# chymaera96/GraFP

Measured on AMD Instinct MI355X. Metric: clips/sec contrastive step @ batch 1024, higher is better.
Workload: dtype bf16; 1 GPU; contrastive step at global batch 1024 (1024 pairs/GPU x 1 GPU, global negatives), 1 s clips @16 kHz, mel->kNN-graph->GNN->NT-Xent, fwd+bwd+Adam, random-init GraphEncoder-t (18.4M params); global_batch=1024, parallelism=dp1, k=3

## Files before the change

### grafp_amd/_lib.py

```python
import ctypes
import os
import subprocess

import torch

_HERE = os.path.dirname(os.path.abspath(__file__))
LIB_PATH = os.environ.get("GRAFP_HIP_LIB") or os.path.join(_HERE, "libgrafp_hip.so")
HEADER_PATH = os.path.join(os.path.dirname(_HERE), "include", "grafp_hip.h")

_c = ctypes
_P = _c.c_void_p
_I = _c.c_int
_L = _c.c_int64
_Z = _c.c_size_t
_F = _c.c_float

SIGNATURES = {
    "grafp_abi_version": (_I, []),
    "grafp_last_error": (_c.c_char_p, []),
    "grafp_logmel_f32": (_I, [_P, _L, _I, _I, _I, _I, _I, _P, _P, _P, _P, _P, _P, _P]),
    "grafp_unfold_segments_f32": (_I, [_P, _I, _I, _I, _I, _P, _P]),
    "grafp_stream_logmel_f32": (_I, [_P, _P, _P, _P, _P, _P, _P, _I, _I, _I, _I, _I, _I, _P, _P, _P, _P, _P, _P, _P]),
    "grafp_stream_segments_f32": (_I, [_P, _P, _P, _I, _I, _I, _I, _I, _I, _P, _P]),
    "grafp_peak_extract_fwd_f32": (_I, [_P, _I, _I, _I, _P, _P, _I, _I, _I, _I, _P, _P, _P, _P]),
    "grafp_peak_extract_bwd_f32": (_I, [_P, _I, _I, _I, _I, _I, _I, _I, _P, _P, _P, _P, _P, _P, _P, _Z, _P]),
    "grafp_peak_extract_bwd_workspace": (_Z, [_I, _I, _I, _I]),
    "grafp_knn_graph_workspace": (_Z, [_I, _I, _I]),
    "grafp_knn_normalize_f32": (_I, [_P, _I, _I, _I, _I, _P, _P, _P]),
    "grafp_knn_topk_f32": (_I, [_P, _P, _I, _I, _I, _I, _P, _P]),
    "grafp_knn_topk_i32": (_I, [_P, _P, _I, _I, _I, _I, _P, _P]),
    "grafp_knn_normalize_strided": (_I, [_P, _I, _L, _L, _I, _I, _I, _I, _P, _P, _P]),
    "grafp_knn_graph_f32": (_I, [_P, _I, _I, _I, _I, _I, _P, _P, _Z, _P]),
    "grafp_knn_pre_supported": (_I, [_I, _I, _I]),
    "grafp_knn_pre_workspace": (_Z, [_I, _I, _I]),
    "grafp_knn_graph_pre": (_I, [_P, _I, _L, _L, _I, _I, _I, _I, _I, _P, _I, _P, _Z, _P]),
    "grafp_knn_split_supported": (_I, [_I, _I, _I]),
    "grafp_knn_split_preferred": (_I, [_I, _I, _I]),
    "grafp_knn_split_workspace": (_Z, [_I, _I, _I]),
    "grafp_knn_split_preferred_for": (_I, [_I, _I, _I, _I]),
    "grafp_knn_split_workspace_for": (_Z, [_I, _I, _I, _I]),
    "grafp_knn_graph_split": (_I, [_P, _I, _L, _L, _I, _I, _I, _I, _P, _I, _P, _Z, _P, _P]),
    "grafp_mrconv_fwd_f32": (_I, [_P, _P, _I, _I, _I, _I, _P, _P]),
    "grafp_mrconv_bwd_f32": (_I, [_P, _P, _P, _I, _I, _I, _I, _P, _P]),
    "grafp_mrconv_fwd_strided": (_I, [_P, _I, _L, _L, _P, _I, _I, _I, _I, _P, _L, _L, _P]),
    "grafp_mrconv_bwd_strided": (_I, [_P, _I, _L, _L, _P, _P, _L, _L, _I, _I, _I, _I, _P, _P]),
    "grafp_mrconv_fwd_strided_i32": (_I, [_P, _I, _L, _L, _P, _I, _I, _I, _I, _P, _L, _L, _P]),
    "grafp_mrconv_bwd_strided_i32": (_I, [_P, _I, _L, _L, _P, _P, _L, _L, _I, _I, _I, _I, _P, _P]),
    "grafp_mrconv_arg_supported": (_I, [_I, _L, _L, _L, _L, _I, _I]),
    "grafp_mrconv_fwd_arg": (_I, [_P, _I, _L, _L, _P, _I, _I, _I, _I, _I, _P, _L, _L, _P, _P]),
    "grafp_mrconv_bwd_arg": (_I, [_P, _I, _P, _I, _P, _L, _L, _I, _I, _I, _I, _P, _L, _L, _P]),
    "grafp_mrconv_plan": (_I, [_I, _L, _L, _L, _L, _I, _I, _I, _I, _I, _I, _I, _P]),
    "grafp_stride2_taps_fwd": (_I, [_P, _I, _L, _I, _P, _P]),
    "grafp_stride2_taps_bwd": (_I, [_P, _I, _L, _I, _P, _P]),
    "grafp_bn_workspace": (_Z, [_I, _L]),
    "grafp_bn_fwd": (_I, [_P, _I, _I, _L, _I, _P, _P, _P, _P, _I, _F, _F, _F, _I, _P, _P, _P, _P, _P, _P, _Z, _P]),
    "grafp_bn_bwd": (_I, [_P, _P, _I, _I, _L, _I, _P, _P, _P, _P, _P, _I, _F, _I, _P, _P, _P, _P, _P, _Z, _P]),
    "grafp_bn_sync_bytes": (_Z, [_I, _L]),
    "grafp_bn_fwd_1pass": (_I, [_P, _I, _I, _L, _I, _P, _P, _P, _P, _I, _F, _F, _F, _I, _P, _P, _P, _P, _P, _P, _Z, _P, _I, _P]),
    "grafp_bn_bwd_1pass": (_I, [_P, _P, _I, _I, _L, _I, _P, _P, _P, _P, _P, _I, _F, _I, _P, _P, _P, _P, _P, _Z, _P, _I, _P]),
    "grafp_bn_plan": (_I, [_I, _I, _L, _I, _I, _I, _I, _I, _P]),
    "grafp_ivfpq_scan_f32": (_I, [_P, _I, _I, _P, _I, _P, _I, _P, _P, _P, _I, _P, _L, _P, _P, _P]),
    "grafp_pq_assign_f32": (_I, [_P, _L, _I, _I, _P, _P, _P, _I, _P, _P, _P]),
    "grafp_kmeans_workspace": (_Z, [_L, _I, _I, _I]),
    "grafp_kmeans_f32": (_I, [_P, _L, _I, _I, _P, _P, _P, _I, _I, _P, _P, _Z, _P]),
    "grafp_ivfpq_probe_f32": (_I, [_P, _I, _I, _P, _I, _I, _P, _P]),
    "grafp_ivfpq_search_f32": (_I, [_P, _I, _I, _P, _I, _P, _I, _P, _P, _P, _P, _I, _I, _P, _P, _P]),
    "grafp_debug_occupy": (_I, [_I, _I, _L, _P]),
    "grafp_conv1x1_gemm_supported": (_I, [_I, _I, _I, _L, _I]),
    "grafp_conv1x1_gemm_partials": (_I, [_I, _I, _I, _L, _I]),
    "grafp_conv1x1_gemm_plan": (_I, [_I, _I, _I, _L, _I, _P]),
    "grafp_conv1x1_gemm_bf16": (_I, [_P, _P, _I, _I, _I, _L, _I, _P, _I, _F, _P, _P, _P]),
    "grafp_conv1x1_gemm_affine_bf16": (_I, [_P, _P, _I, _I, _I, _L, _I, _P, _I, _F, _P, _P]),
    "grafp_conv1x1_gemm_cat_bf16": (_I, [_P, _P, _I, _P, _I, _I, _L, _P, _P]),
    "grafp_split_bf16_planes": (_I, [_P, _L, _P, _P, _P]),
    "grafp_conv1x1_gemm_split_f32": (_I, [_P, _P, _I, _I, _L, _P, _P]),
    "grafp_weights_prepare": (_I, [_P, _P, _I, _P]),
    "grafp_bn_finalize": (_I, [_P, _I, _I, _I, _L, _I, _P, _P, _P, _F, _F, _I, _P, _P, _P, _P, _P, _P]),
    "grafp_bn_affine_bf16": (_I, [_P, _I, _L, _I, _P, _P, _I, _F, _P, _P]),
    "grafp_bn_finalize_affine_bf16": (_I, [_P, _P, _I, _I, _I, _L, _I, _P, _P, _P, _F, _F, _P, _P, _P, _P, _P, _P, _I, _F, _P, _P]),
    "grafp_conv1x1_wgrad_workspace": (_Z, [_I, _I, _I, _L]),
    "grafp_conv1x1_wgrad_bf16": (_I, [_P, _P, _I, _I, _I, _L, _P, _P, _Z, _P]),
    "grafp_conv1x1_wgrad_pro_workspace": (_Z, [_I, _I, _I, _L, _I]),
    "grafp_conv1x1_wgrad_plan": (_I, [_I, _I, _I, _L, _I, _P]),
    "grafp_conv1x1_wgrad_pro_bf16": (_I, [_P, _P, _I, _I, _I, _L, _I, _P, _I, _F, _P, _P, _Z, _P]),
# ... 93 lines not shown
```

### grafp_amd/csrc/mrconv.hip

```cpp
#include <math.h>

#define GRAFP_STORE_FAMILY 3
#include "elemio.h"

namespace grafp {

constexpr int MR_THREADS = 256;

__device__ __forceinline__ int clampi(int64_t v, int n) {
    return v < 0 ? 0 : (v >= n ? n - 1 : (int)v);
}

template <typename T> constexpr int MR_NPAR = sizeof(T) == 4 ? 2 : 4;

__device__ __forceinline__ unsigned long long mr_fix_encode(float g, float scale) {
    const float v = __builtin_rintf(g * scale);
    const float hf = __builtin_truncf(v * 9.5367431640625e-7f);
    const float lf = __builtin_fmaf(hf, -1048576.0f, v);
    const int hi = (int)hf, lo = (int)lf;
    return ((unsigned long long)(unsigned)(hi + (lo >> 31)) << 32) | (unsigned long long)(unsigned)lo;
}
__device__ __forceinline__ float mr_fix_decode(unsigned long long a) {
    const int lo = (int)(unsigned)a;
    const int hi = (int)(unsigned)(a >> 32) - (lo >> 31);
    return (float)__builtin_fma((double)hi, 1048576.0, (double)lo);
}
struct MrScale {
    float scale, inv_scale;
    bool poisoned;
    __device__ __forceinline__ unsigned long long encode(float g) const { return mr_fix_encode(g, scale); }
    __device__ __forceinline__ float out(float base, unsigned long long acc) const {
        return poisoned ? NAN : base + mr_fix_decode(acc) * inv_scale;
    }
};
__device__ __forceinline__ void mr_scale_publish(unsigned m, unsigned *s_max, int tid) {
#pragma unroll
    for (int o = 32; o > 0; o >>= 1) m = max(m, (unsigned)__shfl_xor((int)m, o));
    if ((tid & 63) == 0) s_max[tid >> 6] = m;
}
__device__ __forceinline__ MrScale mr_scale_read(const unsigned *s_max) {
    const unsigned mbits = max(max(s_max[0], s_max[1]), max(s_max[2], s_max[3]));
    MrScale s;
    s.poisoned = mbits >= 0x7f800000u;
    int ex = 0;
    (void)frexpf(__uint_as_float(mbits), &ex);
    int sh = mbits ? 39 - ex : 0;
    sh = sh > 100 ? 100 : sh;
    s.scale = ldexpf(1.0f, sh);
    s.inv_scale = ldexpf(1.0f, -sh);
    return s;
}

__device__ __forceinline__ bool mr_first_max(int k, float v, float &best) {
    const bool wins = k == 0 || v > best;
    if (wins) best = v;
    return wins;
}

#define MR_WALK(V, tid, N, c, n)                    \
    int c = ((tid) * (V)) / (N), n = ((tid) * (V)) - c * (N)
#define MR_NEXT(V, N, c, n)                         \
    do {                                            \
        n += MR_THREADS * (V);                      \
        while (n >= (N)) { n -= (N); ++c; }         \
    } while (0)
// ... 289 lines not shown
#pragma unroll
        for (int it = 0; it < MRB_ITEMS; ++it) {
            if (pc[it] < cc) {
                const float *row = rows + pc[it] * N;
                float best[4] = {-INFINITY, -INFINITY, -INFINITY, -INFINITY};
                int bj[4];
                for (int k = 0; k < K; ++k) {
                    const int4 j4 = *reinterpret_cast<const int4 *>(sidx + k * N + pn[it]);
                    const int jj[4] = {j4.x, j4.y, j4.z, j4.w};
#pragma unroll
                    for (int e = 0; e < 4; ++e)
                        if (mr_first_max(k, row[jj[e]] - xi[it][e], best[e])) bj[e] = jj[e];
                }
                if (!fx.poisoned) {
#pragma unroll
                    for (int e = 0; e < 4; ++e)
                        atomicAdd(reinterpret_cast<unsigned long long *>(&acc[pc[it] * N + bj[e]]), fx.encode(godd[it][e]));
                }
            }
        }
        __syncthreads();
#pragma unroll
        for (int it = 0; it < MRB_ITEMS; ++it)
            if (pc[it] < cc) {
                float v[4];
#pragma unroll
                for (int e = 0; e < 4; ++e)
                    v[e] = fx.out(base[it][e], (unsigned long long)acc[pc[it] * N + pn[it] + e]);
                ElemIO<T>::store(db + (size_t)(c0 + pc[it]) * x_sc + pn[it], v, false);
            }
    }
}

template <typename T, typename I>
__global__ __launch_bounds__(MR_THREADS) void mrconv_bwd_a_kernel(const unsigned char *__restrict__ arg,
                                                                  const I *__restrict__ idx,
                                                                  const T *__restrict__ gout, int64_t g_sb,
                                                                  int64_t g_sc, T *__restrict__ dx, int64_t d_sb,
                                                                  int64_t d_sc, int C, int N, int K, int CC, int plain) {
    extern __shared__ __attribute__((aligned(16))) char smem[];
    __shared__ unsigned s_max[MR_THREADS / 64];
    const int b = blockIdx.y, tid = threadIdx.x;
    unsigned long long *acc = reinterpret_cast<unsigned long long *>(smem);
    int *sidx = reinterpret_cast<int *>(acc + MRB_SLAB);
    const int nslab = (C + CC - 1) / CC;
    int off[MRB_ITEMS], pn[MRB_ITEMS], pc[MRB_ITEMS];
    mr_pieces(tid, N, pc, pn);
#pragma unroll
    for (int it = 0; it < MRB_ITEMS; ++it) off[it] = pc[it] * N + pn[it];
    const T *ge_p[MRB_ITEMS];
    T *dx_p[MRB_ITEMS];
    const unsigned char *ar_p[MRB_ITEMS];
    const int64_t cstep = (int64_t)gridDim.x * CC;
#pragma unroll
    for (int it = 0; it < MRB_ITEMS; ++it) {
        const int64_t c = (int64_t)blockIdx.x * CC + pc[it];
        ge_p[it] = gout + (size_t)b * g_sb + (size_t)(2 * c) * g_sc + pn[it];
        dx_p[it] = dx + (size_t)b * d_sb + (size_t)c * d_sc + pn[it];
        ar_p[it] = arg + ((size_t)b * C + c) * (N / 4) + pn[it] / 4;
    }
    const int64_t ge_step = 2 * cstep * g_sc, dx_step = cstep * d_sc, ar_step = cstep * (N / 4);
    typedef typename ElemIO<T>::Raw4 Raw;
    constexpr int NPAR = MR_NPAR<T>;
    Raw pe[NPAR][MRB_ITEMS], po[NPAR][MRB_ITEMS];
    unsigned pa[NPAR][MRB_ITEMS];
    auto fetch = [&](int par, int slab) {
        const int cc = min(CC, C - slab * CC);
#pragma unroll
        for (int it = 0; it < MRB_ITEMS; ++it) {
            if (pc[it] < cc) {
                pe[par][it] = GRAFP_LD_ONCE(16, reinterpret_cast<const Raw *>(ge_p[it]));
                po[par][it] = GRAFP_LD_ONCE(16, reinterpret_cast<const Raw *>(ge_p[it] + g_sc));
                pa[par][it] = *ar_p[it];
            }
            ge_p[it] += ge_step;
            ar_p[it] += ar_step;
        }
    };
    int slab = blockIdx.x;
    const int G = gridDim.x;
#pragma unroll
    for (int par = 0; par < NPAR; ++par)
        if (slab + par * G < nslab) fetch(par, slab + par * G);
    stage_idx<I>(sidx, idx + (size_t)b * N * K, N, K, tid);
    while (slab < nslab) {
#pragma unroll
        for (int par = 0; par < NPAR; ++par) {
            if (slab < nslab) {
                const int cc = min(CC, C - slab * CC);
                __syncthreads();
                float godd[MRB_ITEMS][4], base[MRB_ITEMS][4];
                unsigned ak[MRB_ITEMS];
                unsigned m = 0;
#pragma unroll
                for (int it = 0; it < MRB_ITEMS; ++it)
                    if (pc[it] < cc) {
                        ak[it] = pa[par][it];
                        *reinterpret_cast<uint4 *>(acc + off[it]) = make_uint4(0, 0, 0, 0);
                        *reinterpret_cast<uint4 *>(acc + off[it] + 2) = make_uint4(0, 0, 0, 0);
                        float ge[4];
                        ElemIO<T>::unpack(pe[par][it], ge);
                        ElemIO<T>::unpack(po[par][it], godd[it]);
#pragma unroll
                        for (int e = 0; e < 4; ++e) {
                            base[it][e] = ge[e] - godd[it][e];
                            m = max(m, __float_as_uint(godd[it][e]) & 0x7fffffffu);
                        }
                    }
                mr_scale_publish(m, s_max, tid);
                __syncthreads();
                if (slab + NPAR * G < nslab) fetch(par, slab + NPAR * G);
                const MrScale fx = mr_scale_read(s_max);
                if (!fx.poisoned) {
#pragma unroll
                    for (int it = 0; it < MRB_ITEMS; ++it)
                        if (pc[it] < cc) {
                            unsigned long long *arow = acc + (off[it] - pn[it]);
                            int bj[4] = {0, 0, 0, 0};
                            for (int k = 0; k < K; ++k) {
                                const int4 j4 = *reinterpret_cast<const int4 *>(sidx + k * N + pn[it]);
                                const int jj[4] = {j4.x, j4.y, j4.z, j4.w};
#pragma unroll
                                for (int e = 0; e < 4; ++e) bj[e] = ((ak[it] >> (2 * e)) & 3u) == (unsigned)k ? jj[e] : bj[e];
                            }
#pragma unroll
                            for (int e = 0; e < 4; ++e) atomicAdd(arow + bj[e], fx.encode(godd[it][e]));
                        }
                }
                __syncthreads();
#pragma unroll
                for (int it = 0; it < MRB_ITEMS; ++it) {
                    if (pc[it] < cc) {
                        float v[4];
                        const uint4 a01 = *reinterpret_cast<const uint4 *>(acc + off[it]);
                        const uint4 a23 = *reinterpret_cast<const uint4 *>(acc + off[it] + 2);
                        const unsigned long long a[4] = {((unsigned long long)a01.y << 32) | a01.x,
                                                         ((unsigned long long)a01.w << 32) | a01.z,
                                                         ((unsigned long long)a23.y << 32) | a23.x,
                                                         ((unsigned long long)a23.w << 32) | a23.z};
#pragma unroll
                        for (int e = 0; e < 4; ++e) v[e] = fx.out(base[it][e], a[e]);
                        ElemIO<T>::store(dx_p[it], v, plain != 0);
                    }
                    dx_p[it] += dx_step;
                }
                slab += G;
            }
        }
    }
}

enum { MR_PATH_PERSISTENT = 0, MR_PATH_VEC4 = 1, MR_PATH_SCALAR = 2, MR_PATH_RECORD = 3 };
struct MrLaunch {
    int path;
    int items;
    int cc;
    int nslab, per_clip;
    size_t lds;
};
constexpr size_t MR_LDS_LIMIT = 160 * 1024;
constexpr int MR_FWD_ELEMS = 4096;
static_assert(MRB_SLAB <= MRP_SLAB, "a row that fits the backward slab fits the forward one");

static inline int mr_clamp_cc(int cc, int C) { return cc < 1 ? 1 : (cc > C ? C : cc); }

static int mr_choose(int64_t x_sb, int64_t x_sc, int64_t o_sb, int64_t o_sc, int N, int K, int C, int B,
                     bool aligned, bool backward, bool with_arg, MrLaunch *L) {
    const bool v4 = aligned && N % 4 == 0 && x_sb % 4 == 0 && x_sc % 4 == 0 && o_sb % 4 == 0 && o_sc % 4 == 0;
    const size_t edges = (size_t)K * N;
    const size_t lds_fwd_p = (MRP_SLAB + edges) * 4, lds_bwd_p = (3 * (size_t)MRB_SLAB + edges) * 4,
                 lds_bwd_a = (2 * (size_t)MRB_SLAB + edges) * 4;
    auto lds_generic = [&](int cc) {
        const size_t slab = (size_t)cc * N;
        return (backward ? 4 * ((slab + 1) & ~(size_t)1) + edges : slab + edges) * 4;
    };
    const bool record = with_arg && v4 && K <= 4 && N <= MRB_SLAB && lds_fwd_p <= MR_LDS_LIMIT && lds_bwd_a <= MR_LDS_LIMIT;
    const int slab = backward ? MRB_SLAB : MRP_SLAB;
    const size_t lds_p = !backward ? lds_fwd_p : (record ? lds_bwd_a : lds_bwd_p);
// ... 6 lines not shown
    }
    int items = 0, cc = mr_clamp_cc(MR_FWD_ELEMS / N, C);
    if (backward) {
        const int per_item = MR_THREADS * (v4 ? 4 : 1);
        items = N <= 2 * per_item ? 2 : 8;
        cc = mr_clamp_cc(items * per_item / N, C);
        GRAFP_REQUIRE((size_t)cc * N <= (size_t)items * per_item, "mrconv_bwd: N=%d exceeds the %d nodes a workgroup covers", N,
                      items * per_item);
        while (cc > 1 && lds_generic(cc) > MR_LDS_LIMIT) --cc;
    }
    GRAFP_REQUIRE(lds_generic(cc) <= MR_LDS_LIMIT, "mrconv_%s: N=%d K=%d needs %zu B of LDS (> 160 KiB)",
                  backward ? "bwd" : "fwd", N, K, lds_generic(cc));
    *L = {v4 ? MR_PATH_VEC4 : MR_PATH_SCALAR, items, cc, (C + cc - 1) / cc, (C + cc - 1) / cc, lds_generic(cc)};
    return GRAFP_OK;
}

static int mr_check_args(const char *op, bool pointers, int dtype, int B, int C, int N, int K) {
    GRAFP_REQUIRE(pointers, "%s: null pointer", op);
    GRAFP_REQUIRE(B > 0 && C > 0 && N > 0 && K > 0, "%s: bad shape B=%d C=%d N=%d K=%d", op, B, C, N, K);
    GRAFP_REQUIRE(dtype == GRAFP_F32 || dtype == GRAFP_BF16, "%s: dtype %d not in {f32, bf16}", op, dtype);
    return GRAFP_OK;
}

static bool mr_aligned(int dtype, const void *a, const void *b, const void *c = nullptr) {
    return (((uintptr_t)a | (uintptr_t)b | (uintptr_t)c) % (dtype == GRAFP_F32 ? 16 : 8)) == 0;
}

template <typename Kern, typename... Args>
static int mr_launch(const char *name, Kern kern, const MrLaunch &L, int B, grafp_stream_t stream, Args... args) {
    (void)hipFuncSetAttribute((const void *)kern, hipFuncAttributeMaxDynamicSharedMemorySize, (int)L.lds);
    hipLaunchKernelGGL(kern, dim3(L.per_clip, B), dim3(MR_THREADS), L.lds, (hipStream_t)stream, args...);
    GRAFP_CHECK_LAUNCH(name);
    return GRAFP_OK;
}

}

static int mrconv_fwd_impl(const char *op, const void *x, int dtype, int64_t x_sb, int64_t x_sc, const void *idx, int idx32,
                           int B, int C, int N, int K, void *out, int64_t o_sb, int64_t o_sc, grafp_stream_t stream,
                           unsigned char *arg = nullptr) {
    using namespace grafp;
    if (int e = mr_check_args(op, x && idx && out, dtype, B, C, N, K)) return e;
    MrLaunch L;
    if (int e = mr_choose(x_sb, x_sc, o_sb, o_sc, N, K, C, B, mr_aligned(dtype, x, out), false, arg != nullptr, &L)) return e;
    GRAFP_REQUIRE(!arg || L.path == MR_PATH_RECORD,
                  "mrconv_fwd_arg: shape / alignment outside grafp_mrconv_arg_supported (N=%d K=%d)", N, K);
    int rc = GRAFP_OK;
    for_elem_idx(dtype, idx32, [&](auto te, auto ti) {
        using T = typename decltype(te)::type;
        using I = typename decltype(ti)::type;
        if (L.path == MR_PATH_PERSISTENT || L.path == MR_PATH_RECORD) {
            const int plain = plain_stores((size_t)2 * B * C * N * sizeof(T), "GRAFP_MR_PLAIN_MAX_MB", 140);
            for_bool(arg != nullptr, [&](auto wk) {
                rc = mr_launch("mrconv_fwd_p_kernel", mrconv_fwd_p_kernel<T, I, decltype(wk)::value>, L, B, stream, (const T *)x,
                               x_sb, x_sc, (const I *)idx, (T *)out, o_sb, o_sc, C, N, K, L.cc, arg, plain);
            });
        } else {
            for_bool(L.path == MR_PATH_VEC4, [&](auto vec) {
                rc = mr_launch("mrconv_fwd_kernel", mrconv_fwd_kernel<T, decltype(vec)::value ? 4 : 1, I>, L, B, stream,
                               (const T *)x, x_sb, x_sc, (const I *)idx, (T *)out, o_sb, o_sc, C, N, K, L.cc);
            });
        }
    });
    return rc;
}

static int mrconv_bwd_impl(const char *op, const void *x, const unsigned char *arg, int dtype, int64_t x_sb, int64_t x_sc,
                           const void *idx, int idx32, const void *grad_out, int64_t g_sb, int64_t g_sc, int B, int C, int N,
                           int K, void *dx, grafp_stream_t stream) {
    using namespace grafp;
    if (int e = mr_check_args(op, (x || arg) && idx && grad_out && dx, dtype, B, C, N, K)) return e;
    MrLaunch L;
    if (int e = mr_choose(x_sb, x_sc, g_sb, g_sc, N, K, C, B, mr_aligned(dtype, x, grad_out, dx), true, arg != nullptr, &L)) return e;
    GRAFP_REQUIRE(!arg || L.path == MR_PATH_RECORD,
                  "mrconv_bwd_arg: shape / alignment outside grafp_mrconv_arg_supported (N=%d K=%d)", N, K);
    int rc = GRAFP_OK;
    for_elem_idx(dtype, idx32, [&](auto te, auto ti) {
        using T = typename decltype(te)::type;
        using I = typename decltype(ti)::type;
        if (L.path == MR_PATH_RECORD) {
            const int plain = plain_stores((size_t)B * C * N * sizeof(T), "GRAFP_MR_PLAIN_MAX_MB", 140);
            rc = mr_launch("mrconv_bwd_a_kernel", mrconv_bwd_a_kernel<T, I>, L, B, stream, arg, (const I *)idx,
                           (const T *)grad_out, g_sb, g_sc, (T *)dx, x_sb, x_sc, C, N, K, L.cc, plain);
        } else if (L.path == MR_PATH_PERSISTENT) {
            rc = mr_launch("mrconv_bwd_p_kernel", mrconv_bwd_p_kernel<T, I>, L, B, stream, (const T *)x, x_sb, x_sc,
                           (const I *)idx, (const T *)grad_out, g_sb, g_sc, (T *)dx, C, N, K, L.cc);
        } else {
            for_bool(L.path == MR_PATH_VEC4, [&](auto vec) {
                for_bool(L.items == 2, [&](auto two) {
                    rc = mr_launch("mrconv_bwd_kernel",
                                   mrconv_bwd_kernel<T, decltype(vec)::value ? 4 : 1, I, decltype(two)::value ? 2 : 8>, L, B,
                                   stream, (const T *)x, x_sb, x_sc, (const I *)idx, (const T *)grad_out, g_sb, g_sc, (T *)dx,
                                   C, N, K, L.cc);
                });
            });
        }
    });
    return rc;
}

extern "C" int grafp_mrconv_fwd_strided(const void *x, int dtype, int64_t x_sb, int64_t x_sc, const int64_t *idx, int B,
                                        int C, int N, int K, void *out, int64_t o_sb, int64_t o_sc,
                                        grafp_stream_t stream) {
    return mrconv_fwd_impl("mrconv_fwd", x, dtype, x_sb, x_sc, idx, 0, B, C, N, K, out, o_sb, o_sc, stream);
}
extern "C" int grafp_mrconv_fwd_strided_i32(const void *x, int dtype, int64_t x_sb, int64_t x_sc, const int32_t *idx,
                                            int B, int C, int N, int K, void *out, int64_t o_sb, int64_t o_sc,
                                            grafp_stream_t stream) {
    return mrconv_fwd_impl("mrconv_fwd", x, dtype, x_sb, x_sc, idx, 1, B, C, N, K, out, o_sb, o_sc, stream);
}
extern "C" int grafp_mrconv_bwd_strided(const void *x, int dtype, int64_t x_sb, int64_t x_sc, const int64_t *idx,
                                        const void *grad_out, int64_t g_sb, int64_t g_sc, int B, int C, int N, int K,
                                        void *dx, grafp_stream_t stream) {
    return mrconv_bwd_impl("mrconv_bwd", x, nullptr, dtype, x_sb, x_sc, idx, 0, grad_out, g_sb, g_sc, B, C, N, K, dx, stream);
}
extern "C" int grafp_mrconv_bwd_strided_i32(const void *x, int dtype, int64_t x_sb, int64_t x_sc, const int32_t *idx,
// ... 47 lines not shown
```

### grafp_amd/encoder/graph_encoder.py

```python
import contextlib

import torch
import torch.nn.functional as F
from torch import nn

from .. import ops
from ._dense import (bn_act, conv1x1, conv_bn_act, deferred_counters, deferred_norm, from_cbn, shortcut_token,
                     stride2_operands, to_cbn)
from .gcn_lib.torch_nn import act_layer
from .gcn_lib.torch_vertex import Grapher

_SIZES = {
    "t": ([2, 2, 6, 2], [64, 128, 256, 512]),
    "s": ([2, 2, 6, 2], [80, 160, 400, 640]),
    "m": ([2, 2, 16, 2], [96, 192, 384, 768]),
}


class Downsample(nn.Module):

    def __init__(self, in_dim=3, out_dim=768):
        super().__init__()
        self.conv = nn.Sequential(nn.Conv2d(in_dim, out_dim, 3, stride=2, padding=1), nn.BatchNorm2d(out_dim))

# ... 86 lines not shown
    @contextlib.contextmanager
    def one_weight_preparation(self):
        if self._lowp_hold is not None:
            yield
            return
        self._lowp_hold = False
        try:
            yield
        finally:
            self._lowp_hold = None

    def forward(self, x, views=1):
        x = to_cbn(x)
        g = int(views)
        if torch.is_autocast_enabled() and x.is_cuda:
            if self._lowp is None:
                self._lowp = ops.lowp_weights([m for m in self.modules() if isinstance(m, nn.Conv2d)
                                               and m.kernel_size == (1, 1) and m is not self.proj])
            if not self._lowp_hold:
                self._lowp.refresh(torch.get_autocast_dtype("cuda"))
                if self._lowp_hold is not None:
                    self._lowp_hold = True
        elif self._lowp is not None:
            self._lowp.clear()
        with deferred_counters():
            x = conv_bn_act(self.stem[0], self.stem[1], x, act=ops.ACT_LEAKY, slope=self.stem[2].negative_slope,
                            groups=g)
            for mod in self.backbone:
                if isinstance(mod, Downsample):
                    x = mod.forward_cbn(x, g)
                else:
                    x = mod[1].forward_cbn(mod[0].forward_cbn(x, g), g)
        with torch.autocast(x.device.type, enabled=False):
            pooled = x.float().mean(dim=2)
            w = self.proj.weight.reshape(self.proj.out_channels, -1)
            h = torch.mm(w.float(), pooled) + self.proj.bias.float().reshape(-1, 1)
        return h.t().contiguous()
```

### grafp_amd/ops.py

```python
import collections
import contextlib
import ctypes
import math
import os

import numpy as np
import torch
from torch.amp import custom_bwd, custom_fwd

from ._lib import check, lib

_vp = ctypes.c_void_p


def _require_gpu(*tensors):
    for t in tensors:
        if t is not None and not t.is_cuda:
            raise RuntimeError(
                "grafp_amd ops run only on a HIP device (MI355X): got a CPU tensor and there is no CPU "
                "fallback by design (the CPU restatement lives in oracle/ and is test infrastructure).")


def _p(t):
    return _vp(t.data_ptr()) if t is not None else None
# ... 664 lines not shown
                                               N, K, _p(out), o_sb, o_sc, _p(arg), _stream()), "mrconv_fwd_arg")
            ctx.save_for_backward(arg, idx)
            return out
        fwd = lib.grafp_mrconv_fwd_strided_i32 if idx.dtype == torch.int32 else lib.grafp_mrconv_fwd_strided
        with _timed("mrconv_fwd", (B, C, N, K)):
            check(fwd(_p(x), _DT[x.dtype], sb, sc, _p(idx), B, C, N, K, _p(out), o_sb, o_sc, _stream()), "mrconv_fwd")
        ctx.save_for_backward(x, idx)
        return out

    @staticmethod
    def backward(ctx, grad_out):
        x, idx = ctx.saved_tensors
        layout = ctx.layout
        B, C, N, shape, dtype = ctx.dims
        K = idx.shape[-1]
        g = grad_out.detach().to(dtype).contiguous()
        g_sb, g_sc = (2 * C * N, N) if layout == "bcn" else (N, B * N)
        sb, sc = (C * N, N) if layout == "bcn" else (N, B * N)
        if ctx.from_arg:
            dx = torch.empty(shape, dtype=dtype, device=g.device)
            with _timed("mrconv_bwd", (B, C, N, K)):
                check(lib.grafp_mrconv_bwd_arg(_p(x), _DT[dtype], _p(idx), int(idx.dtype == torch.int32), _p(g), g_sb,
                                               g_sc, B, C, N, K, _p(dx), sb, sc, _stream()), "mrconv_bwd_arg")
            return dx, None, None
        dx = torch.empty_like(x)
        with _timed("mrconv_bwd", (B, C, N, K)):
            bwd = lib.grafp_mrconv_bwd_strided_i32 if idx.dtype == torch.int32 else lib.grafp_mrconv_bwd_strided
            check(bwd(_p(x), _DT[x.dtype], sb, sc, _p(idx), _p(g), g_sb, g_sc, B, C, N, K, _p(dx), _stream()), "mrconv_bwd")
        return dx, None, None


def max_relative(x, idx, layout="bcn"):
    return _MaxRelative.apply(x, idx, layout)


ACT_NONE, ACT_RELU, ACT_LEAKY = 0, 1, 2


_BN_SYNC = {}


def _bn_sync(device, C, M):
    if switches.bn_two_pass:
        return None
    key = (device, _raw_stream(device.index if device.index is not None else _cur_device()))
    buf = _BN_SYNC.get(key)
    need = int(lib.grafp_bn_sync_bytes(C, M))
    if buf is None or buf.numel() * 8 < need:
        buf = torch.full((max(1 << 18, (need + 7) // 8),), -1, dtype=torch.int64, device=device)
        _BN_SYNC[key] = buf
    return buf


class _BnAct(torch.autograd.Function):
    @staticmethod
    def forward(ctx, x, gamma, beta, pre_bias, residual, running_mean, running_var, training, momentum, eps, act,
                slope, groups):
        _require_gpu(x, gamma, beta)
        if x.dtype not in _DT:
            x = x.float()
        x = x.detach().contiguous()
        C = x.shape[0]
        M = x.numel() // C
        res = None if residual is None else residual.detach().to(x.dtype).contiguous()
        g32, b32 = _f32c(gamma), _f32c(beta)
        pb = None if pre_bias is None else _f32c(pre_bias)
# ... 1482 lines not shown
```

### include/grafp_hip.h

```cpp
#ifndef GRAFP_HIP_H
#define GRAFP_HIP_H

#include <stddef.h>
#include <stdint.h>

#ifdef __cplusplus
extern "C" {
#endif

#define GRAFP_OK 0
#define GRAFP_ERR_ARG (-1)
#define GRAFP_ERR_WORKSPACE (-2)
#define GRAFP_ERR_LAUNCH (-3)

#define GRAFP_ABI_VERSION 1
#define GRAFP_KNN_MAX_K 8
#define GRAFP_SEARCH_MAX_K 32

typedef void *grafp_stream_t;

#define GRAFP_F32 0
#define GRAFP_BF16 1

int grafp_abi_version(void);
// ... 44 lines not shown

int grafp_knn_split_supported(int C, int N, int k);
int grafp_knn_split_preferred(int C, int N, int k);
int grafp_knn_split_preferred_for(int dtype, int C, int N, int k);
size_t grafp_knn_split_workspace(int B, int C, int N);
size_t grafp_knn_split_workspace_for(int dtype, int B, int C, int N);
int grafp_knn_graph_split(const void *x, int dtype, int64_t stride_b, int64_t stride_c, int B, int C, int N, int k,
                          void *idx, int idx_is_i32, void *ws, size_t ws_bytes, int32_t *n_uncertified,
                          grafp_stream_t stream);

int grafp_mrconv_fwd_f32(const float *x, const int64_t *idx, int B, int C, int N, int K, float *out,
                         grafp_stream_t stream);
int grafp_mrconv_bwd_f32(const float *x, const int64_t *idx, const float *grad_out, int B, int C, int N, int K,
                         float *dx, grafp_stream_t stream);
int grafp_mrconv_fwd_strided(const void *x, int dtype, int64_t x_sb, int64_t x_sc, const int64_t *idx, int B, int C,
                             int N, int K, void *out, int64_t o_sb, int64_t o_sc, grafp_stream_t stream);
int grafp_mrconv_bwd_strided(const void *x, int dtype, int64_t x_sb, int64_t x_sc, const int64_t *idx,
                             const void *grad_out, int64_t g_sb, int64_t g_sc, int B, int C, int N, int K, void *dx,
                             grafp_stream_t stream);

int grafp_mrconv_fwd_strided_i32(const void *x, int dtype, int64_t x_sb, int64_t x_sc, const int32_t *idx, int B, int C,
                                 int N, int K, void *out, int64_t o_sb, int64_t o_sc, grafp_stream_t stream);
int grafp_mrconv_bwd_strided_i32(const void *x, int dtype, int64_t x_sb, int64_t x_sc, const int32_t *idx,
                                 const void *grad_out, int64_t g_sb, int64_t g_sc, int B, int C, int N, int K,
                                 void *dx, grafp_stream_t stream);
int grafp_mrconv_arg_supported(int dtype, int64_t x_sb, int64_t x_sc, int64_t o_sb, int64_t o_sc, int N, int K);
int grafp_mrconv_fwd_arg(const void *x, int dtype, int64_t x_sb, int64_t x_sc, const void *idx, int idx_is_i32, int B,
                         int C, int N, int K, void *out, int64_t o_sb, int64_t o_sc, uint8_t *arg, grafp_stream_t stream);
int grafp_mrconv_bwd_arg(const uint8_t *arg, int dtype, const void *idx, int idx_is_i32, const void *grad_out,
                         int64_t g_sb, int64_t g_sc, int B, int C, int N, int K, void *dx, int64_t d_sb, int64_t d_sc,
                         grafp_stream_t stream);
int grafp_mrconv_plan(int dtype, int64_t x_sb, int64_t x_sc, int64_t o_sb, int64_t o_sc, int B, int C, int N, int K,
                      int aligned, int backward, int with_arg, int *info);

size_t grafp_bn_workspace(int C, int64_t M);
int grafp_bn_fwd(const void *x, int dtype, int C, int64_t M, int groups, const float *pre_bias, const float *gamma,
                 const float *beta, const void *residual, int act, float slope, float eps, float momentum,
                 int training, float *running_mean, float *running_var, void *out, float *save_mean,
                 float *save_invstd, void *ws, size_t ws_bytes, grafp_stream_t stream);
int grafp_bn_bwd(const void *x, const void *dz, int dtype, int C, int64_t M, int groups, const float *pre_bias,
                 const float *gamma,
                 const float *beta, const float *save_mean, const float *save_invstd, int act, float slope,
                 int training, void *dx, float *dgamma, float *dbeta, float *dpre_bias , void *ws,
                 size_t ws_bytes, grafp_stream_t stream);
size_t grafp_bn_sync_bytes(int C, int64_t M);
int grafp_bn_fwd_1pass(const void *x, int dtype, int C, int64_t M, int groups, const float *pre_bias,
                       const float *gamma, const float *beta, const void *residual, int act, float slope, float eps,
                       float momentum, int training, float *running_mean, float *running_var, void *out,
                       float *save_mean, float *save_invstd, void *ws, size_t ws_bytes, int32_t *sync, int spin_limit,
                       grafp_stream_t stream);
int grafp_bn_bwd_1pass(const void *x, const void *dz, int dtype, int C, int64_t M, int groups, const float *pre_bias,
                       const float *gamma, const float *beta, const float *save_mean, const float *save_invstd,
                       int act, float slope, int training, void *dx, float *dgamma, float *dbeta,
                       float *dpre_bias , void *ws, size_t ws_bytes, int32_t *sync, int spin_limit,
                       grafp_stream_t stream);
int grafp_bn_plan(int dtype, int C, int64_t M, int groups, int training, int backward, int aligned, int have_sync,
                  int *info);

int grafp_ivfpq_scan_f32(const float *q, int nq, int d, const float *centroids, int nlist, const float *codebooks,
                         int M, const uint8_t *codes, const int64_t *list_start, const int32_t *probe, int nprobe,
                         const int64_t *out_start, int64_t row_stride, float *out_dist, int32_t *out_pos,
                         grafp_stream_t stream);

int grafp_pq_assign_f32(const float *x, int64_t n, int D, int G, const float *base ,
                        const int32_t *base_idx , const float *cent , int k,
                        int32_t *out , uint8_t *out_u8 , grafp_stream_t stream);
// ... 225 lines not shown
```

Before: 11230 clips/s.

## Add fused node-mean pooling kernels and restructure max-relative backward scatter

Adds a HIP node_mean forward/backward kernel pair that replaces the float-cast-then-mean pooling with a single pass that reads bf16 directly and writes an f32 mean, avoiding a materialized f32 copy. It also reworks the mrconv record-path backward kernel: K is now a template parameter, neighbor selection uses bitfield-select instead of a K-loop compare, the shared accumulator is zeroed once and re-zeroed after readout, and the next slab's scale max is published one iteration early to drop a barrier. The trade-offs are more template instantiations and extra LDS space for a double-buffered scale, plus a bf16 rounding correction in the pooling backward.

```diff
diff --git a/grafp_amd/_lib.py b/grafp_amd/_lib.py
--- a/grafp_amd/_lib.py
+++ b/grafp_amd/_lib.py
@@ -50,6 +50,8 @@
     "grafp_mrconv_fwd_arg": (_I, [_P, _I, _L, _L, _P, _I, _I, _I, _I, _I, _P, _L, _L, _P, _P]),
     "grafp_mrconv_bwd_arg": (_I, [_P, _I, _P, _I, _P, _L, _L, _I, _I, _I, _I, _P, _L, _L, _P]),
     "grafp_mrconv_plan": (_I, [_I, _L, _L, _L, _L, _I, _I, _I, _I, _I, _I, _I, _P]),
+    "grafp_node_mean": (_I, [_P, _I, _I, _I, _I, _P, _P]),
+    "grafp_node_mean_bwd": (_I, [_P, _I, _I, _I, _I, _P, _P]),
     "grafp_stride2_taps_fwd": (_I, [_P, _I, _L, _I, _P, _P]),
     "grafp_stride2_taps_bwd": (_I, [_P, _I, _L, _I, _P, _P]),
     "grafp_bn_workspace": (_Z, [_I, _L]),
diff --git a/grafp_amd/csrc/mrconv.hip b/grafp_amd/csrc/mrconv.hip
--- a/grafp_amd/csrc/mrconv.hip
+++ b/grafp_amd/csrc/mrconv.hip
@@ -30,7 +30,10 @@
     bool poisoned;
     __device__ __forceinline__ unsigned long long encode(float g) const { return mr_fix_encode(g, scale); }
     __device__ __forceinline__ float out(float base, unsigned long long acc) const {
-        return poisoned ? NAN : base + mr_fix_decode(acc) * inv_scale;
+        return poisoned ? NAN : sum(base, acc);
+    }
+    __device__ __forceinline__ float sum(float base, unsigned long long acc) const {
+        return base + mr_fix_decode(acc) * inv_scale;
     }
 };
 __device__ __forceinline__ void mr_scale_publish(unsigned m, unsigned *s_max, int tid) {
@@ -386,22 +389,62 @@
     }
 }
 
-template <typename T, typename I>
+template <typename T> struct MrAbsMax;
+template <> struct MrAbsMax<float> {
+    unsigned m = 0;
+    __device__ __forceinline__ void add(const float4 &t) {
+        m = max(max(m, __float_as_uint(t.x) & 0x7fffffffu), __float_as_uint(t.y) & 0x7fffffffu);
+        m = max(max(m, __float_as_uint(t.z) & 0x7fffffffu), __float_as_uint(t.w) & 0x7fffffffu);
+    }
+    __device__ __forceinline__ unsigned bits() const { return m; }
+};
+template <> struct MrAbsMax<unsigned short> {
+    typedef unsigned short us2 __attribute__((ext_vector_type(2)));
+    us2 m = {0, 0};
+    __device__ __forceinline__ void add(const uint2 &t) {
+        m = __builtin_elementwise_max(m, __builtin_bit_cast(us2, t.x & 0x7fff7fffu));
+        m = __builtin_elementwise_max(m, __builtin_bit_cast(us2, t.y & 0x7fff7fffu));
+    }
+    __device__ __forceinline__ unsigned bits() const { return (unsigned)max(m.x, m.y) << 16; }
+};
+
+__device__ __forceinline__ int mr_sel(int mask, int a, int b) {
+    int r;
+    asm("v_bfi_b32 %0, %1, %2, %3" : "=v"(r) : "v"(mask), "v"(a), "v"(b));
+    return r;
+}
+template <int KK>
+__device__ __forceinline__ int mr_pick(unsigned rec, int sh, const int (&j)[4]) {
+    if (KK == 1) return j[0];
+    const int b0 = __builtin_amdgcn_sbfe((int)rec, sh, 1);
+    const int lo = mr_sel(b0, j[1], j[0]);
+    if (KK == 2) return lo;
+    const int b1 = __builtin_amdgcn_sbfe((int)rec, sh + 1, 1);
+    return mr_sel(b1, KK == 3 ? j[2] : mr_sel(b0, j[3], j[2]), lo);
+}
+
+template <typename T, typename I, int KK>
 __global__ __launch_bounds__(MR_THREADS) void mrconv_bwd_a_kernel(const unsigned char *__restrict__ arg,
                                                                   const I *__restrict__ idx,
                                                                   const T *__restrict__ gout, int64_t g_sb,
                                                                   int64_t g_sc, T *__restrict__ dx, int64_t d_sb,
-                                                                  int64_t d_sc, int C, int N, int K, int CC, int plain) {
+                                                                  int64_t d_sc, int C, int N, int CC, int plain) {
     extern __shared__ __attribute__((aligned(16))) char smem[];
-    __shared__ unsigned s_max[MR_THREADS / 64];
+    __shared__ unsigned s_max[2][MR_THREADS / 64];
     const int b = blockIdx.y, tid = threadIdx.x;
     unsigned long long *acc = reinterpret_cast<unsigned long long *>(smem);
     int *sidx = reinterpret_cast<int *>(acc + MRB_SLAB);
     const int nslab = (C + CC - 1) / CC;
-    int off[MRB_ITEMS], pn[MRB_ITEMS], pc[MRB_ITEMS];
+    int pn[MRB_ITEMS], pc[MRB_ITEMS];
     mr_pieces(tid, N, pc, pn);
-#pragma unroll
-    for (int it = 0; it < MRB_ITEMS; ++it) off[it] = pc[it] * N + pn[it];
+    unsigned long long *own[MRB_ITEMS], *arow[MRB_ITEMS];
+    const int *edge[MRB_ITEMS];
+#pragma unroll
+    for (int it = 0; it < MRB_ITEMS; ++it) {
+        arow[it] = acc + pc[it] * N;
+        own[it] = arow[it] + pn[it];
+        edge[it] = sidx + pn[it];
+    }
     const T *ge_p[MRB_ITEMS];
     T *dx_p[MRB_ITEMS];
     const unsigned char *ar_p[MRB_ITEMS];
@@ -416,6 +459,7 @@
     const int64_t ge_step = 2 * cstep * g_sc, dx_step = cstep * d_sc, ar_step = cstep * (N / 4);
     typedef typename ElemIO<T>::Raw4 Raw;
     constexpr int NPAR = MR_NPAR<T>;
+    static_assert(NPAR % 2 == 0, "the halves of s_max alternate with the slots");
     Raw pe[NPAR][MRB_ITEMS], po[NPAR][MRB_ITEMS];
     unsigned pa[NPAR][MRB_ITEMS];
     auto fetch = [&](int par, int slab) {
@@ -431,73 +475,84 @@
             ar_p[it] += ar_step;
         }
     };
+    auto publish_max = [&](int par, int slab) {
+        const int cc = min(CC, C - slab * CC);
+        MrAbsMax<T> m;
+#pragma unroll
+        for (int it = 0; it < MRB_ITEMS; ++it)
+            if (pc[it] < cc) m.add(po[par][it]);
+        mr_scale_publish(m.bits(), s_max[par & 1], tid);
+    };
     int slab = blockIdx.x;
     const int G = gridDim.x;
 #pragma unroll
     for (int par = 0; par < NPAR; ++par)
         if (slab + par * G < nslab) fetch(par, slab + par * G);
-    stage_idx<I>(sidx, idx + (size_t)b * N * K, N, K, tid);
+#pragma unroll
+    for (int it = 0; it < MRB_ITEMS; ++it) {
+        *reinterpret_cast<uint4 *>(acc + (tid + it * MR_THREADS) * 4) = make_uint4(0, 0, 0, 0);
+        *reinterpret_cast<uint4 *>(acc + (tid + it * MR_THREADS) * 4 + 2) = make_uint4(0, 0, 0, 0);
+    }
+    stage_idx<I>(sidx, idx + (size_t)b * N * KK, N, KK, tid);
+    if (slab < nslab) publish_max(0, slab);
+    __syncthreads();
     while (slab < nslab) {
 #pragma unroll
         for (int par = 0; par < NPAR; ++par) {
             if (slab < nslab) {
                 const int cc = min(CC, C - slab * CC);
-                __syncthreads();
+                const MrScale fx = mr_scale_read(s_max[par & 1]);
                 float godd[MRB_ITEMS][4], base[MRB_ITEMS][4];
                 unsigned ak[MRB_ITEMS];
-                unsigned m = 0;
 #pragma unroll
                 for (int it = 0; it < MRB_ITEMS; ++it)
                     if (pc[it] < cc) {
                         ak[it] = pa[par][it];
-                        *reinterpret_cast<uint4 *>(acc + off[it]) = make_uint4(0, 0, 0, 0);
-                        *reinterpret_cast<uint4 *>(acc + off[it] + 2) = make_uint4(0, 0, 0, 0);
                         float ge[4];
                         ElemIO<T>::unpack(pe[par][it], ge);
                         ElemIO<T>::unpack(po[par][it], godd[it]);
 #pragma unroll
-                        for (int e = 0; e < 4; ++e) {
-                            base[it][e] = ge[e] - godd[it][e];
-                            m = max(m, __float_as_uint(godd[it][e]) & 0x7fffffffu);
-                        }
+                        for (int e = 0; e < 4; ++e) base[it][e] = ge[e] - godd[it][e];
                     }
-                mr_scale_publish(m, s_max, tid);
-                __syncthreads();
                 if (slab + NPAR * G < nslab) fetch(par, slab + NPAR * G);
-                const MrScale fx = mr_scale_read(s_max);
+                if (slab + G < nslab) publish_max((par + 1) % NPAR, slab + G);
                 if (!fx.poisoned) {
 #pragma unroll
                     for (int it = 0; it < MRB_ITEMS; ++it)
                         if (pc[it] < cc) {
-                            unsigned long long *arow = acc + (off[it] - pn[it]);
-                            int bj[4] = {0, 0, 0, 0};
-                            for (int k = 0; k < K; ++k) {
-                                const int4 j4 = *reinterpret_cast<const int4 *>(sidx + k * N + pn[it]);
-                                const int jj[4] = {j4.x, j4.y, j4.z, j4.w};
-#pragma unroll
-                                for (int e = 0; e < 4; ++e) bj[e] = ((ak[it] >> (2 * e)) & 3u) == (unsigned)k ? jj[e] : bj[e];
+                            int jj[4][4];
+#pragma unroll
+                            for (int k = 0; k < KK; ++k) {
+                                const int4 j4 = *reinterpret_cast<const int4 *>(edge[it] + k * N);
+                                jj[0][k] = j4.x; jj[1][k] = j4.y; jj[2][k] = j4.z; jj[3][k] = j4.w;
                             }
 #pragma unroll
-                            for (int e = 0; e < 4; ++e) atomicAdd(arow + bj[e], fx.encode(godd[it][e]));
+                            for (int e = 0; e < 4; ++e)
+                                atomicAdd(arow[it] + mr_pick<KK>(ak[it], 2 * e, jj[e]), fx.encode(godd[it][e]));
                         }
                 }
                 __syncthreads();
 #pragma unroll
                 for (int it = 0; it < MRB_ITEMS; ++it) {
                     if (pc[it] < cc) {
-                        float v[4];
-                        const uint4 a01 = *reinterpret_cast<const uint4 *>(acc + off[it]);
-                        const uint4 a23 = *reinterpret_cast<const uint4 *>(acc + off[it] + 2);
-                        const unsigned long long a[4] = {((unsigned long long)a01.y << 32) | a01.x,
-                                                         ((unsigned long long)a01.w << 32) | a01.z,
-                                                         ((unsigned long long)a23.y << 32) | a23.x,
-                                                         ((unsigned long long)a23.w << 32) | a23.z};
-#pragma unroll
-                        for (int e = 0; e < 4; ++e) v[e] = fx.out(base[it][e], a[e]);
+                        float v[4] = {NAN, NAN, NAN, NAN};
+                        if (!fx.poisoned) {
+                            const uint4 a01 = *reinterpret_cast<const uint4 *>(own[it]);
+                            const uint4 a23 = *reinterpret_cast<const uint4 *>(own[it] + 2);
+                            *reinterpret_cast<uint4 *>(own[it]) = make_uint4(0, 0, 0, 0);
+                            *reinterpret_cast<uint4 *>(own[it] + 2) = make_uint4(0, 0, 0, 0);
+                            const unsigned long long a[4] = {((unsigned long long)a01.y << 32) | a01.x,
+                                                             ((unsigned long long)a01.w << 32) | a01.z,
+                                                             ((unsigned long long)a23.y << 32) | a23.x,
+                                                             ((unsigned long long)a23.w << 32) | a23.z};
+#pragma unroll
+                            for (int e = 0; e < 4; ++e) v[e] = fx.sum(base[it][e], a[e]);
+                        }
                         ElemIO<T>::store(dx_p[it], v, plain != 0);
                     }
                     dx_p[it] += dx_step;
                 }
+                __syncthreads();
                 slab += G;
             }
         }
@@ -570,6 +625,13 @@
     hipLaunchKernelGGL(kern, dim3(L.per_clip, B), dim3(MR_THREADS), L.lds, (hipStream_t)stream, args...);
     GRAFP_CHECK_LAUNCH(name);
     return GRAFP_OK;
+}
+
+template <typename F> static inline void for_k4(int K, F &&f) {
+    if (K == 1) f(std::integral_constant<int, 1>{});
+    else if (K == 2) f(std::integral_constant<int, 2>{});
+    else if (K == 3) f(std::integral_constant<int, 3>{});
+    else f(std::integral_constant<int, 4>{});
 }
 
 }
@@ -618,8 +680,10 @@
         using I = typename decltype(ti)::type;
         if (L.path == MR_PATH_RECORD) {
             const int plain = plain_stores((size_t)B * C * N * sizeof(T), "GRAFP_MR_PLAIN_MAX_MB", 140);
-            rc = mr_launch("mrconv_bwd_a_kernel", mrconv_bwd_a_kernel<T, I>, L, B, stream, arg, (const I *)idx,
-                           (const T *)grad_out, g_sb, g_sc, (T *)dx, x_sb, x_sc, C, N, K, L.cc, plain);
+            for_k4(K, [&](auto kk) {
+                rc = mr_launch("mrconv_bwd_a_kernel", mrconv_bwd_a_kernel<T, I, decltype(kk)::value>, L, B, stream, arg,
+                               (const I *)idx, (const T *)grad_out, g_sb, g_sc, (T *)dx, x_sb, x_sc, C, N, L.cc, plain);
+            });
         } else if (L.path == MR_PATH_PERSISTENT) {
             rc = mr_launch("mrconv_bwd_p_kernel", mrconv_bwd_p_kernel<T, I>, L, B, stream, (const T *)x, x_sb, x_sc,
                            (const I *)idx, (const T *)grad_out, g_sb, g_sc, (T *)dx, C, N, K, L.cc);
diff --git a/grafp_amd/csrc/pool.hip b/grafp_amd/csrc/pool.hip
--- /dev/null
+++ b/grafp_amd/csrc/pool.hip
@@ -0,0 +1,131 @@
+#include "elemio.h"
+
+namespace grafp {
+
+constexpr int POOL_THREADS = 256;
+constexpr int POOL_MAX_BLOCKS = 65536;
+
+template <int W> __device__ __forceinline__ float pool_piece_sum(const float (&e)[W]) {
+    if constexpr (W == 8) return ((e[0] + e[1]) + (e[2] + e[3])) + ((e[4] + e[5]) + (e[6] + e[7]));
+    else if constexpr (W == 4) return (e[0] + e[1]) + (e[2] + e[3]);
+    else return e[0];
+}
+
+template <typename T, int W>
+__global__ __launch_bounds__(POOL_THREADS) void node_mean_kernel(const T *__restrict__ x, float *__restrict__ out,
+                                                                 int64_t R, int N, int L) {
+    const int lane = threadIdx.x & 63, j = lane & (L - 1), rows_per_wave = 64 / L;
+    const int64_t wave = (int64_t)blockIdx.x * (POOL_THREADS / 64) + (threadIdx.x >> 6);
+    const int64_t step = (int64_t)gridDim.x * (POOL_THREADS / 64) * rows_per_wave;
+    const int nv = N / W;
+    const float n = (float)N;
+    for (int64_t r0 = wave * rows_per_wave; r0 < R; r0 += step) {
+        const int64_t r = r0 + lane / L;
+        float s = 0.0f;
+        if (r < R) {
+            const T *row = x + r * N;
+            for (int v = j; v < nv; v += L) {
+                float e[W];
+                if constexpr (W == 1) e[0] = ElemIO<T>::ld1(row + v); else ElemIO<T>::load(row + (size_t)v * W, e);
+                s += pool_piece_sum<W>(e);
+            }
+        }
+        for (int o = L >> 1; o > 0; o >>= 1) s += __shfl_xor(s, o);
+        if (j == 0 && r < R) out[r] = s / n;
+    }
+}
+
+template <typename T> __device__ __forceinline__ float pool_quotient(float g, float n) {
+    float q = g / n;
+    if constexpr (sizeof(T) == 2) {
+        unsigned u = __float_as_uint(q);
+        const float rem = fmaf(-q, n, g);
+        if ((u & 0xffffu) == 0x8000u && rem != 0.0f && (u & 0x7f800000u) != 0x7f800000u)
+            u = ((rem > 0.0f) == (q > 0.0f)) ? u | 1u : u - 1u;
+        q = __uint_as_float(u);
+    }
+    return q;
+}
+
+template <typename T, int W>
+__global__ __launch_bounds__(POOL_THREADS) void node_mean_bwd_kernel(const float *__restrict__ g, T *__restrict__ dx,
+                                                                     int64_t R, int N, int L, int plain) {
+    const int lane = threadIdx.x & 63, j = lane & (L - 1), rows_per_wave = 64 / L;
+    const int64_t wave = (int64_t)blockIdx.x * (POOL_THREADS / 64) + (threadIdx.x >> 6);
+    const int64_t step = (int64_t)gridDim.x * (POOL_THREADS / 64) * rows_per_wave;
+    const int nv = N / W;
+    const float n = (float)N;
+    for (int64_t r = wave * rows_per_wave + lane / L; r < R; r += step) {
+        const float q = pool_quotient<T>(g[r], n);
+        T *row = dx + r * N;
+        if constexpr (W == 1) {
+            for (int v = j; v < nv; v += L) ElemIO<T>::st1(row + v, q);
+        } else {
+            float e[W];
+#pragma unroll
+            for (int i = 0; i < W; ++i) e[i] = q;
+            for (int v = j; v < nv; v += L) ElemIO<T>::store(row + (size_t)v * W, e, plain != 0);
+        }
+    }
+}
+
+struct PoolLaunch {
+    bool vec;
+    int lanes;
+    int blocks;
+};
+static PoolLaunch pool_choose(int dtype, int64_t R, int N, const void *act) {
+    const int W = dtype == GRAFP_F32 ? 4 : 8;
+    PoolLaunch P;
+    P.vec = N % W == 0 && (uintptr_t)act % 16 == 0;
+    const int nv = P.vec ? N / W : N;
+    P.lanes = 1;
+    while (P.lanes < 64 && P.lanes < nv) P.lanes <<= 1;
+    const int64_t rows_per_block = (int64_t)(POOL_THREADS / 64) * (64 / P.lanes);
+    const int64_t blocks = (R + rows_per_block - 1) / rows_per_block;
+    P.blocks = (int)(blocks < POOL_MAX_BLOCKS ? blocks : POOL_MAX_BLOCKS);
+    return P;
+}
+static int pool_check_args(const char *op, bool pointers, int dtype, int C, int B, int N) {
+    GRAFP_REQUIRE(pointers, "%s: null pointer", op);
+    GRAFP_REQUIRE(C > 0 && B > 0 && N > 0 && N < (1 << 24), "%s: bad shape C=%d B=%d N=%d", op, C, B, N);
+    GRAFP_REQUIRE(dtype == GRAFP_F32 || dtype == GRAFP_BF16, "%s: dtype %d not in {f32, bf16}", op, dtype);
+    return GRAFP_OK;
+}
+
+}
+
+extern "C" int grafp_node_mean(const void *x, int dtype, int C, int B, int N, float *out, grafp_stream_t stream) {
+    using namespace grafp;
+    if (int e = pool_check_args("node_mean", x && out, dtype, C, B, N)) return e;
+    const int64_t R = (int64_t)C * B;
+    const PoolLaunch P = pool_choose(dtype, R, N, x);
+    for_elem(dtype, [&](auto te) {
+        using T = typename decltype(te)::type;
+        for_bool(P.vec, [&](auto vec) {
+            constexpr int W = decltype(vec)::value ? ElemIO<T>::W : 1;
+            hipLaunchKernelGGL((node_mean_kernel<T, W>), dim3(P.blocks), dim3(POOL_THREADS), 0, (hipStream_t)stream,
+                               (const T *)x, out, R, N, P.lanes);
+        });
+    });
+    GRAFP_CHECK_LAUNCH("node_mean_kernel");
+    return GRAFP_OK;
+}
+
+extern "C" int grafp_node_mean_bwd(const float *g, int dtype, int C, int B, int N, void *dx, grafp_stream_t stream) {
+    using namespace grafp;
+    if (int e = pool_check_args("node_mean_bwd", g && dx, dtype, C, B, N)) return e;
+    const int64_t R = (int64_t)C * B;
+    const PoolLaunch P = pool_choose(dtype, R, N, dx);
+    for_elem(dtype, [&](auto te) {
+        using T = typename decltype(te)::type;
+        const int plain = plain_stores((size_t)R * N * sizeof(T), "GRAFP_POOL_PLAIN_MAX_MB", 140);
+        for_bool(P.vec, [&](auto vec) {
+            constexpr int W = decltype(vec)::value ? ElemIO<T>::W : 1;
+            hipLaunchKernelGGL((node_mean_bwd_kernel<T, W>), dim3(P.blocks), dim3(POOL_THREADS), 0, (hipStream_t)stream, g,
+                               (T *)dx, R, N, P.lanes, plain);
+        });
+    });
+    GRAFP_CHECK_LAUNCH("node_mean_bwd_kernel");
+    return GRAFP_OK;
+}
diff --git a/grafp_amd/encoder/graph_encoder.py b/grafp_amd/encoder/graph_encoder.py
--- a/grafp_amd/encoder/graph_encoder.py
+++ b/grafp_amd/encoder/graph_encoder.py
@@ -142,7 +142,7 @@
                 else:
                     x = mod[1].forward_cbn(mod[0].forward_cbn(x, g), g)
         with torch.autocast(x.device.type, enabled=False):
-            pooled = x.float().mean(dim=2)
+            pooled = ops.node_mean(x) if x.is_cuda else x.float().mean(dim=2)
             w = self.proj.weight.reshape(self.proj.out_channels, -1)
             h = torch.mm(w.float(), pooled) + self.proj.bias.float().reshape(-1, 1)
         return h.t().contiguous()
diff --git a/grafp_amd/ops.py b/grafp_amd/ops.py
--- a/grafp_amd/ops.py
+++ b/grafp_amd/ops.py
@@ -720,6 +720,44 @@
 
 def max_relative(x, idx, layout="bcn"):
     return _MaxRelative.apply(x, idx, layout)
+
+
+def _node_mean_args(x):
+    if x.dim() != 3:
+        raise ValueError(f"node_mean: x must be (C, B, N), got shape {tuple(x.shape)}")
+    if x.dtype not in _DT:
+        raise TypeError(f"node_mean: dtype {x.dtype} not in {{float32, bfloat16}}")
+    if 0 in x.shape:
+        raise ValueError(f"node_mean: empty activation {tuple(x.shape)}")
+    if x.shape[2] >= 1 << 24:
+        raise ValueError(f"node_mean: N={x.shape[2]} is not below 2^24")
+    _require_gpu(x)
+
+
+class _NodeMean(torch.autograd.Function):
+    @staticmethod
+    def forward(ctx, x):
+        _node_mean_args(x)
+        x = x.detach().contiguous()
+        C, B, N = x.shape
+        ctx.dims = (C, B, N, x.dtype)
+        out = torch.empty((C, B), dtype=torch.float32, device=x.device)
+        with _timed("node_mean", (C, B, N)):
+            check(lib.grafp_node_mean(_p(x), _DT[x.dtype], C, B, N, _p(out), _stream()), "node_mean")
+        return out
+
+    @staticmethod
+    def backward(ctx, g):
+        C, B, N, dtype = ctx.dims
+        g = _f32c(g)
+        dx = torch.empty((C, B, N), dtype=dtype, device=g.device)
+        with _timed("node_mean", (C, B, N)):
+            check(lib.grafp_node_mean_bwd(_p(g), _DT[dtype], C, B, N, _p(dx), _stream()), "node_mean_bwd")
+        return dx
+
+
+def node_mean(x):
+    return _NodeMean.apply(x)
 
 
 ACT_NONE, ACT_RELU, ACT_LEAKY = 0, 1, 2
diff --git a/include/grafp_hip.h b/include/grafp_hip.h
--- a/include/grafp_hip.h
+++ b/include/grafp_hip.h
@@ -100,6 +100,9 @@
                          grafp_stream_t stream);
 int grafp_mrconv_plan(int dtype, int64_t x_sb, int64_t x_sc, int64_t o_sb, int64_t o_sc, int B, int C, int N, int K,
                       int aligned, int backward, int with_arg, int *info);
+
+int grafp_node_mean(const void *x, int dtype, int C, int B, int N, float *out, grafp_stream_t stream);
+int grafp_node_mean_bwd(const float *g, int dtype, int C, int B, int N, void *dx, grafp_stream_t stream);
 
 size_t grafp_bn_workspace(int C, int64_t M);
 int grafp_bn_fwd(const void *x, int dtype, int C, int64_t M, int groups, const float *pre_bias, const float *gamma,
```

Result: no change. 11310 clips/s, median of 6 (+0.8%).
